# materight/non-rigid-object-tracking

Measured on NVIDIA B200. Metric: PC masker frames/sec at 1080p, higher is better.
Workload: dtype u8/f64

## Files before the change

non-rigid-object-tracking_b200/csrc/pcm_api.cu:

```cuda
#include "../../include/pcm_b200.h"
#include "pcm_kernels.cuh"
#include "pcm_score_variants.h"
#include "pcm_quickshift.cuh"
#include "pcm_forest_fit.cuh"
#include "pcm_prior.cuh"
#include "pcm_slic.cuh"
#include "pcm_host.h"

#include <cudaTypedefs.h>
#include <cub/device/device_radix_sort.cuh>
#include <cub/device/device_scan.cuh>

#include <algorithm>
#include <atomic>
#include <cmath>
#include <cstdarg>
#include <cstddef>
#include <cstdio>
#include <cstring>
#include <cstdlib>
#include <string>
#include <utility>
#include <vector>

// ... 383 lines not shown
    g.PS = (g.RS * (MAX_TILE_H + 2 * n) + 127) / 128 * 128;
    return g;
}

static int int_threshold(double thr) {
    auto le = [&](int v) { return (double)(float)((double)v / 255.0) <= thr; };
    if (!(thr >= -1.0)) return le(-1) ? -1 : -2;
    int t = thr >= 1.5 ? 255 : (int)floor(thr * 255.0);
    t = std::min(std::max(t, -2), 255);
    while (t < 255 && le(t + 1)) ++t;
    while (t >= -1 && !le(t)) --t;
    return t;
}

struct EncTree {
    std::vector<NodeT> nodes;
    std::vector<double> values;
    int n_leaf = 0;
    int depth = 0;
};

struct Encoder {
    const Geom& g;
    const int32_t* feature;
    const double* threshold;
    const int32_t* left;
    const int32_t* right;
    const double* value1;
    int n;
    std::vector<int> tint;
    EncTree out;
    std::string err;

    int skip(int i) const {
        while (left[i] != -1 && tint[i] < -1) i = right[i];
        return i;
    }
    bool run() {
        tint.assign(n, 0);
        for (int i = 0; i < n; ++i) {
            if (left[i] == -1) continue;
            if (left[i] < 0 || left[i] >= n || right[i] < 0 || right[i] >= n) { err = "child index out of range"; return false; }
            if (feature[i] < 0 || feature[i] >= g.F) { err = "feature index out of range"; return false; }
            tint[i] = int_threshold(threshold[i]);
        }
        struct Item { int node, entry, depth; };
        std::vector<Item> queue;
        queue.push_back({skip(0), 0, 0});
        out.nodes.assign(1, make_node(0, 0, 0));
        out.values.assign(1, 0.0);
        const int vplane = 3 * g.n_spaces;
        size_t visited = 0;
        for (size_t qi = 0; qi < queue.size(); ++qi) {
            const Item it = queue[qi];
            if (++visited > (size_t)n + 1) { err = "tree is not a tree"; return false; }
            const int i = it.node;
            if (left[i] == -1) {
                out.nodes[it.entry] = make_node(0u, LEAF_THR, (unsigned)it.entry);
                out.values[it.entry] = value1[i];
                out.n_leaf++;
                out.depth = std::max(out.depth, it.depth);
                continue;
            }
            const int f = feature[i];
            const int q = f / (3 * g.K), rem = f % (3 * g.K), k = rem / 3, ch = rem % 3;
            int dr, dc;
            star_tap(k, dr, dc);
            int plane = 3 * q + ch;
            int thr = tint[i];
            if (thr == -1) { plane = vplane; thr = 0; }
            const unsigned off = (unsigned)(plane * g.PS + (dr + g.n) * g.RS + (dc + g.HX));
            if (off >= (1u << 16)) { err = "tap offset overflow"; return false; }
            const int child = (int)out.nodes.size();
            out.nodes.resize(child + 2, make_node(0, 0, 0));
            out.values.resize(child + 2, 0.0);
            out.nodes[it.entry] = make_node(off, (unsigned)thr, (unsigned)child);
            queue.push_back({skip(left[i]), child, it.depth + 1});
            queue.push_back({skip(right[i]), child + 1, it.depth + 1});
        }
        return true;
    }
};

constexpr int N_SCORE_VARIANTS = 3 * N_SCORE_VARIANTS_PER_PPT;
static const ScoreVariant& score_variant(int i) {
    const ScoreVariant* t = i < N_SCORE_VARIANTS_PER_PPT ? score_variants_ppt6()
                          : i < 2 * N_SCORE_VARIANTS_PER_PPT ? score_variants_ppt7() : score_variants_ppt8();
    return t[i % N_SCORE_VARIANTS_PER_PPT];
}
static const ScoreVariant& pick_score_variant(bool smem, int depth, int ppt) {
    int dyn = -1;
    for (int i = 0; i < N_SCORE_VARIANTS; ++i) {
        const ScoreVariant& v = score_variant(i);
        if (v.smem != smem || v.ppt != ppt) continue;
        if (v.depth == depth) return v;
        if (v.depth == 0) dyn = i;
    }
    return score_variant(dyn);
}

typedef void (*ResidualFn)(const int16_t*, long long, int, int, const double*, const double*, double*);
namespace { extern const ResidualFn pca_residual_kernels[PCM_MAX_PCA_COMPONENTS]; }

struct DeviceShared {
    std::mutex m;
    bool ready = false;
    int sm_count = 0, max_smem_optin = 0;
    PFN_cuTensorMapEncodeTiled_v12000 encode_tiled = nullptr;
    ColorTables h_tables;
    ColorTables* d_tables = nullptr;
};
static DeviceShared& device_shared(int device) {
    static DeviceShared table[64];
    return table[device & 63];
}

extern "C" int pcm_abi_version(void) { return PCM_ABI_VERSION; }
extern "C" const char* pcm_last_error(void) { return g_last_error.c_str(); }

extern "C" int pcm_create(int device, pcm_handle** out) {
    if (!out) return fail(PCM_E_INVALID, "pcm_create: out is NULL");
    *out = nullptr;
    int count = 0;
    cudaError_t e = cudaGetDeviceCount(&count);
    if (e != cudaSuccess || count == 0)
        return fail(PCM_E_CUDA, "pcm_create: no CUDA device (%s); this library has no CPU path",
                    e == cudaSuccess ? "device count 0" : cudaGetErrorString(e));
    if (device < 0 || device >= count) return fail(PCM_E_INVALID, "pcm_create: device %d out of range [0,%d)", device, count);
    CUDA_TRY(cudaSetDevice(device));
    DeviceShared& ds = device_shared(device);
    {
        std::lock_guard<std::mutex> lk(ds.m);
        if (!ds.ready) {
            CUDA_TRY(cudaDeviceGetAttribute(&ds.sm_count, cudaDevAttrMultiProcessorCount, device));
            CUDA_TRY(cudaDeviceGetAttribute(&ds.max_smem_optin, cudaDevAttrMaxSharedMemoryPerBlockOptin, device));
            void* fn = nullptr;
            cudaDriverEntryPointQueryResult qres;
            CUDA_TRY(cudaGetDriverEntryPointByVersion("cuTensorMapEncodeTiled", &fn, 12000, cudaEnableDefault, &qres));
            if (qres != cudaDriverEntryPointSuccess || !fn)
                return fail(PCM_E_CUDA, "pcm_create: driver does not provide cuTensorMapEncodeTiled");
            ds.encode_tiled = reinterpret_cast<PFN_cuTensorMapEncodeTiled_v12000>(fn);
            build_tables(ds.h_tables);
            CUDA_TRY(cudaMalloc(&ds.d_tables, sizeof(ColorTables)));
            CUDA_TRY(cudaMemcpy(ds.d_tables, &ds.h_tables, sizeof(ColorTables), cudaMemcpyHostToDevice));
            for (int i = 0; i < N_SCORE_VARIANTS; ++i)
                CUDA_TRY(cudaFuncSetAttribute(score_variant(i).fn, cudaFuncAttributeMaxDynamicSharedMemorySize, ds.max_smem_optin));
            CUDA_TRY(cudaFuncSetAttribute(qs_density_kernel<false>, cudaFuncAttributeMaxDynamicSharedMemorySize, ds.max_smem_optin));
            CUDA_TRY(cudaFuncSetAttribute(qs_density_kernel<true>, cudaFuncAttributeMaxDynamicSharedMemorySize, ds.max_smem_optin));
            CUDA_TRY(cudaFuncSetAttribute(qs_parent_kernel, cudaFuncAttributeMaxDynamicSharedMemorySize, ds.max_smem_optin));
            CUDA_TRY(cudaFuncSetAttribute(novelty_kernel, cudaFuncAttributeMaxDynamicSharedMemorySize, ds.max_smem_optin));
            for (ResidualFn fn : pca_residual_kernels)
                CUDA_TRY(cudaFuncSetAttribute(fn, cudaFuncAttributeMaxDynamicSharedMemorySize, ds.max_smem_optin));
            ds.ready = true;
        }
    }
    pcm_handle* h = new pcm_handle();
    h->device = device;
    h->sm_count = ds.sm_count;
    h->max_smem_optin = ds.max_smem_optin;
    h->encode_tiled = ds.encode_tiled;
    h->d_tables = ds.d_tables;
    h->h_tables = ds.h_tables;
    CUDA_TRY(cudaStreamCreateWithFlags(&h->own_stream, cudaStreamNonBlocking));
    h->stream = h->own_stream;
    CUDA_TRY(h->err_buf.reserve(sizeof(int)));
    h->d_err = h->err_buf.as<int>();
    CUDA_TRY(cudaMemsetAsync(h->d_err, 0, sizeof(int), h->stream));
    *out = h;
    return PCM_OK;
}

namespace {
const ResidualFn pca_residual_kernels[PCM_MAX_PCA_COMPONENTS] = {
    pca_residual_kernel<1>, pca_residual_kernel<2>, pca_residual_kernel<3>, pca_residual_kernel<4>,
    pca_residual_kernel<5>, pca_residual_kernel<6>, pca_residual_kernel<7>, pca_residual_kernel<8>};
}

// ... 1767 lines not shown
```

non-rigid-object-tracking_b200/csrc/pcm_score.cuh:

```cuda
#pragma once
#include "pcm_device.cuh"
#include <cuda.h>

namespace pcm {

typedef uint2 NodeT;
__host__ __device__ inline NodeT make_node(unsigned tap, unsigned thr, unsigned left) { return make_uint2((tap << 16) | thr, left); }
__host__ __device__ inline unsigned node_tap(const NodeT& n) { return n.x >> 16; }
__host__ __device__ inline unsigned node_thr(const NodeT& n) { return n.x & 0xffffu; }
__host__ __device__ inline unsigned node_left(const NodeT& n) { return n.y; }
__host__ __device__ inline void node_set_left(NodeT& n, unsigned v) { n.y = v; }
constexpr unsigned LEAF_THR = 0xffffu;
constexpr unsigned NODE_BYTES = sizeof(NodeT);

struct DevForest {
    const NodeT* nodes;
    const double* leaves;
    const int4* trees;
    int n_trees, n_nodes, n_leaves;
};

constexpr int MAX_TOP_TREES = 48;
struct TopNodes {
    NodeT n[MAX_TOP_TREES][3];
// ... 117 lines not shown
                    convert((w3[(3 * j) / 4] >> (8 * ((3 * j) % 4))) & 0xff, (w3[(3 * j + 1) / 4] >> (8 * ((3 * j + 1) % 4))) & 0xff,
                            (w3[(3 * j + 2) / 4] >> (8 * ((3 * j + 2) % 4))) & 0xff, j, out);
                    valid |= 1u << (8 * j);
                }
            }
        }
        uint8_t* dst = a.planes + (long long)r * a.pitch + c0;
#pragma unroll
        for (int p = 0; p < NOUT; ++p)
            if (p < nch) *reinterpret_cast<uint32_t*>(dst + p * a.plane_stride) = out[p];
        *reinterpret_cast<uint32_t*>(dst + nch * a.plane_stride) = valid;
        w3[0] = nx[0]; w3[1] = nx[1]; w3[2] = nx[2];
        r = rn; g = gn;
        rn += dr; gn += dg;
        if (gn >= groups_per_row) { gn -= groups_per_row; ++rn; }
    }
    if (a.early) grid_dependency_wait();
}


__device__ __forceinline__ uint32_t smem_u32(const void* p) { return (uint32_t)__cvta_generic_to_shared(p); }

__device__ __forceinline__ void mbar_init(uint32_t bar, uint32_t count) {
    asm volatile("mbarrier.init.shared::cta.b64 [%0], %1;" ::"r"(bar), "r"(count) : "memory");
}
__device__ __forceinline__ void mbar_expect_tx(uint32_t bar, uint32_t bytes) {
    asm volatile("mbarrier.arrive.expect_tx.shared::cta.b64 _, [%0], %1;" ::"r"(bar), "r"(bytes) : "memory");
}
__device__ __forceinline__ void mbar_wait(uint32_t bar, uint32_t parity) {
    uint32_t done;
    do {
        asm volatile(
            "{\n\t.reg .pred p;\n\t"
            "mbarrier.try_wait.parity.shared::cta.b64 p, [%1], %2;\n\t"
            "selp.u32 %0, 1, 0, p;\n\t}"
            : "=r"(done) : "r"(bar), "r"(parity) : "memory");
    } while (!done);
}
__device__ __forceinline__ void tma_load_3d(uint32_t dst, const void* tmap, int x, int y, int z, uint32_t bar) {
    asm volatile(
        "cp.async.bulk.tensor.3d.shared::cluster.global.mbarrier::complete_tx::bytes [%0], [%1, {%2, %3, %4}], [%5];"
        ::"r"(dst), "l"(tmap), "r"(x), "r"(y), "r"(z), "r"(bar) : "memory");
}
__device__ __forceinline__ uint2 lds_v2(uint32_t a) {
    uint2 v;
    asm volatile("ld.shared.v2.u32 {%0, %1}, [%2];" : "=r"(v.x), "=r"(v.y) : "r"(a));
    return v;
}
__device__ __forceinline__ NodeT lds_node(uint32_t a) { return lds_v2(a); }
__device__ __forceinline__ uint32_t lds_u16(uint32_t a) {
    uint32_t v;
    asm volatile("ld.shared.u16 %0, [%1];" : "=r"(v) : "r"(a));
    return v;
}
__device__ __forceinline__ uint32_t lds_u8(uint32_t a) {
    uint32_t v;
    asm volatile("ld.shared.u8 %0, [%1];" : "=r"(v) : "r"(a));
    return v;
}
__device__ __forceinline__ double lds_f64(uint32_t a) {
    double v;
    asm volatile("ld.shared.f64 %0, [%1];" : "=d"(v) : "r"(a));
    return v;
}

struct SegAcc {
    const int32_t* labels;
    int n_labels;
    double thr;
    double* sum;
    double* asum;
    int* area;
    int* rmin;
    int* rmax;
    int* cmin;
    int* cmax;
    int* err;
};

__device__ __forceinline__ double contribution(double p1, double sa, double thr) {
    return __dsub_rn(p1, __dsub_rn(fmax(sa, thr), thr));
}

__device__ __forceinline__ void segment_flush(const SegAcc& s, int lab, double sm, double as, int cnt, int r0, int r1, int col) {
    const int lane = threadIdx.x & 31;
    unsigned todo = __ballot_sync(0xffffffffu, lab >= 0);
    while (todo) {
        const int leader = __ffs(todo) - 1;
        const int L = __shfl_sync(0xffffffffu, lab, leader);
        const bool mine = (lab == L);
        const unsigned members = __ballot_sync(0xffffffffu, mine);
        double x = mine ? sm : 0.0, y = mine ? as : 0.0;
#pragma unroll
        for (int o = 16; o > 0; o >>= 1) {
            x += __shfl_xor_sync(0xffffffffu, x, o);
            y += __shfl_xor_sync(0xffffffffu, y, o);
        }
        const int n = __reduce_add_sync(0xffffffffu, mine ? cnt : 0);
        const int lo = __reduce_min_sync(0xffffffffu, mine ? r0 : 0x7fffffff);
        const int hi = __reduce_max_sync(0xffffffffu, mine ? r1 : -1);
        const int cl = __reduce_min_sync(0xffffffffu, mine ? col : 0x7fffffff);
        const int ch = __reduce_max_sync(0xffffffffu, mine ? col : -1);
        if (lane == leader) {
            atomicAdd(s.sum + L, x);
            atomicAdd(s.asum + L, y);
            atomicAdd(s.area + L, n);
            atomicMin(s.rmin + L, lo);
            atomicMax(s.rmax + L, hi);
            atomicMin(s.cmin + L, cl);
            atomicMax(s.cmax + L, ch);
        }
        todo &= ~members;
    }
}

struct ScoreArgs {
    int cw, ch;
    int tiles_x, tiles_y;
    int tile_y0;
    Geom g;
    unsigned* tile_counter;
    DevForest f0, f1;
    TopNodes top0, top1;
    int depth;
    int blend;
    double w0, w1;
    int novelty;
    DevPCA pca0, pca1;
    double* p1_out;
    double* sa_out;
    SegAcc seg;
    const double* nov_in;
};

__device__ __forceinline__ bool goes_right(uint32_t v, uint32_t x) { return v > (x & 0xffffu); }

__device__ __forceinline__ uint32_t step_child(uint32_t left, uint32_t v, uint32_t x) {
    asm("{\n\t.reg .pred p;\n\t.reg .b32 t;\n\tand.b32 t, %2, 0xffff;\n\tsetp.gt.u32 p, %1, t;\n\t@p add.u32 %0, %0, 8;\n\t}"
        : "+r"(left) : "r"(v), "r"(x));
    return left;
}

template <bool SM, int DEPTH, int PIX_PER_THREAD>
__device__ __forceinline__ void traverse_forest(const uint32_t nodes_s, const uint32_t leaves_s,
                                                const uint8_t* __restrict__ nodes_g,
                                                const uint8_t* __restrict__ leaves_g,
                                                const int4* __restrict__ trees, const int n_trees, const int depth,
                                                const TopNodes& top,
                                                const uint32_t (&pix)[PIX_PER_THREAD],
                                                double (&acc)[PIX_PER_THREAD]) {
    const uint32_t base = SM ? nodes_s : 0u;
    const uint32_t vdelta = leaves_s - nodes_s;

    auto descend = [&](uint32_t (&ref)[PIX_PER_THREAD], const int levels) {
        auto level = [&]() {
            NodeT nd[PIX_PER_THREAD];
            uint32_t v[PIX_PER_THREAD];
#pragma unroll
            for (int g = 0; g < PIX_PER_THREAD; ++g)
                nd[g] = SM ? lds_node(ref[g]) : __ldg(reinterpret_cast<const NodeT*>(nodes_g + ref[g]));
#pragma unroll
            for (int g = 0; g < PIX_PER_THREAD; ++g) v[g] = lds_u8(pix[g] + node_tap(nd[g]));
#pragma unroll
            for (int g = 0; g < PIX_PER_THREAD; ++g) ref[g] = step_child(node_left(nd[g]), v[g], nd[g].x);
        };
        if (DEPTH > 0) {
#pragma unroll
            for (int l = 0; l < levels; ++l) level();
        } else {
#pragma unroll 1
            for (int l = 0; l < levels; ++l) level();
        }
#pragma unroll
        for (int g = 0; g < PIX_PER_THREAD; ++g) {
            const double leaf = SM ? lds_f64(ref[g] + vdelta)
                                   : __ldg(reinterpret_cast<const double*>(leaves_g + ref[g]));
            acc[g] = __dadd_rn(acc[g], leaf);
        }
    };

    const int n_top = n_trees < MAX_TOP_TREES ? n_trees : MAX_TOP_TREES;
    const int rest = DEPTH > 0 ? (DEPTH > 2 ? DEPTH - 2 : 0) : (depth > 2 ? depth - 2 : 0);
#pragma unroll 1
    for (int t = 0; t < n_top; ++t) {
        const NodeT e0 = top.n[t][0], eL = top.n[t][1], eR = top.n[t][2];
        uint32_t ref[PIX_PER_THREAD], v[PIX_PER_THREAD], x1[PIX_PER_THREAD];
#pragma unroll
        for (int g = 0; g < PIX_PER_THREAD; ++g) v[g] = lds_u8(pix[g] + node_tap(e0));
#pragma unroll
        for (int g = 0; g < PIX_PER_THREAD; ++g) {
            const bool right = goes_right(v[g], e0.x);
            x1[g] = right ? eR.x : eL.x;
            ref[g] = (right ? node_left(eR) : node_left(eL)) + base;
        }
#pragma unroll
        for (int g = 0; g < PIX_PER_THREAD; ++g) v[g] = lds_u8(pix[g] + (x1[g] >> 16));
#pragma unroll
        for (int g = 0; g < PIX_PER_THREAD; ++g) ref[g] = step_child(ref[g], v[g], x1[g]);
        descend(ref, DEPTH > 0 ? (DEPTH > 2 ? DEPTH - 2 : 0) : rest);
    }
#pragma unroll 1
    for (int t = n_top; t < n_trees; ++t) {
        uint32_t ref[PIX_PER_THREAD];
#pragma unroll
        for (int g = 0; g < PIX_PER_THREAD; ++g) ref[g] = (uint32_t)trees[t].x + base;
        descend(ref, DEPTH > 0 ? DEPTH : depth);
    }
}

template <int NCH, int PIX_PER_THREAD>
__device__ __forceinline__ void novelty_error(const double* __restrict__ comp, const double* __restrict__ comp255,
                                              const double* __restrict__ mean, const uint32_t* __restrict__ noff,
                                              const double mdc, const int* __restrict__ sp, const Geom& g, const bool interior,
                                              const uint32_t (&pix)[PIX_PER_THREAD], double (&err)[PIX_PER_THREAD]) {
    const int vplane = NCH * g.PS;
    double t[PIX_PER_THREAD];
#pragma unroll
    for (int i = 0; i < PIX_PER_THREAD; ++i) t[i] = 0.0;
#pragma unroll 1
    for (int pass = 0; pass < 2; ++pass) {
#pragma unroll 1
        for (int k = 0; k < g.K; ++k) {
            unsigned ok = (1u << PIX_PER_THREAD) - 1u;
            if (!interior) {
                const int so = sp[k];
                ok = 0;
#pragma unroll
                for (int i = 0; i < PIX_PER_THREAD; ++i) ok |= (unsigned)(lds_u8(pix[i] + vplane + so) != 0) << i;
            }
#pragma unroll
            for (int p = 0; p < NCH; ++p) {
                const int it = k * NCH + p;
                const uint32_t off = noff[it];
                if (pass == 0) {
                    const double c255 = comp255[it];
#pragma unroll
                    for (int i = 0; i < PIX_PER_THREAD; ++i) {
                        const double v = ((ok >> i) & 1u) ? u8_to_double(lds_u8(pix[i] + off)) : -1.0;
                        t[i] = fma(v, c255, t[i]);
                    }
                } else {
                    const double c = comp[it], mu = mean[it];
#pragma unroll
                    for (int i = 0; i < PIX_PER_THREAD; ++i) {
                        const double v = ((ok >> i) & 1u) ? u8_to_double(lds_u8(pix[i] + off)) : -1.0;
                        err[i] += fabs(fma(v, 1.0 / 255.0, -fma(t[i], c, mu)));
                    }
                }
            }
        }
        if (pass == 0) {
#pragma unroll
            for (int i = 0; i < PIX_PER_THREAD; ++i) t[i] -= mdc;
        }
    }
}

__device__ __forceinline__ double blend2(double a, double b, double w0, double w1) {
    return __ddiv_rn(__dadd_rn(__dmul_rn(a, w0), __dmul_rn(b, w1)), __dadd_rn(w0, w1));
}

#ifndef PCM_U8_TILE_BUFS
#define PCM_U8_TILE_BUFS 2
#endif
constexpr int N_TILE_BUF = PCM_U8_TILE_BUFS;

struct ScoreSmem {
    uint32_t tiles, bars, sched, sp, f0_nodes, f0_leaves, f0_trees, f1_nodes, f1_leaves, f1_trees, pca0, pca1, nov_off, total;
};

__host__ __device__ inline uint32_t align_up(uint32_t v, uint32_t a) { return (v + a - 1) / a * a; }

__host__ __device__ inline ScoreSmem score_smem_layout(const Geom& g, const DevForest& f0, const DevForest& f1,
                                                       bool blend, bool novelty, bool forest_smem) {
    ScoreSmem s;
    uint32_t o = 0;
    const int nbuf = N_TILE_BUF;
    s.tiles = o;  o = align_up(o + nbuf * align_up(g.n_planes * g.PS, 128), 128);
    s.bars = o;   o += 8 * nbuf;
    s.sched = o;  o = align_up(o + 4 * nbuf, 16);
    s.sp = o;     o = align_up(o + 4 * g.K, 16);
    s.f0_nodes = s.f0_leaves = s.f1_nodes = s.f1_leaves = 0;
    s.f0_trees = o;  o = align_up(o + 16 * f0.n_trees, 16);
    s.f1_trees = o;
    if (blend) o = align_up(o + 16 * f1.n_trees, 16);
    if (forest_smem) {
        s.f0_nodes = o;  o = align_up(o + NODE_BYTES * f0.n_nodes, 16);
        s.f0_leaves = o; o = align_up(o + 8 * f0.n_nodes, 16);
        if (blend) {
            s.f1_nodes = o;  o = align_up(o + NODE_BYTES * f1.n_nodes, 16);
            s.f1_leaves = o; o = align_up(o + 8 * f1.n_nodes, 16);
        }
    }
    s.pca0 = s.pca1 = s.nov_off = 0;
    if (novelty) {
        s.pca0 = o; o = align_up(o + 24 * g.F, 16);
        if (blend) { s.pca1 = o; o = align_up(o + 24 * g.F, 16); }
        s.nov_off = o; o = align_up(o + 4 * g.F, 16);
    }
    s.total = o;
    return s;
}

template <typename T>
__device__ __forceinline__ void copy_to_smem(T* dst, const T* __restrict__ src, int n) {
    for (int i = threadIdx.x; i < n; i += NTHREADS) dst[i] = src[i];
}

__device__ __forceinline__ void stage_nodes(uint8_t* dst, const NodeT* __restrict__ src, int n) {
    const uint32_t base = smem_u32(dst);
    for (int i = threadIdx.x; i < n; i += NTHREADS) {
        NodeT nd = src[i];
        node_set_left(nd, node_left(nd) + base);
        reinterpret_cast<NodeT*>(dst)[i] = nd;
    }
}

template <bool FOREST_SMEM, int DEPTH, int PIX_PER_THREAD>
__global__ void __launch_bounds__(NTHREADS, PCM_MIN_CTAS) score_kernel(const __grid_constant__ CUtensorMap tmap, const ScoreArgs a) {
    extern __shared__ __align__(128) uint8_t smem[];
    const Geom& g = a.g;
    const ScoreSmem L = score_smem_layout(g, a.f0, a.f1, a.blend != 0, a.novelty != 0 && !a.nov_in, FOREST_SMEM);
    constexpr int TILE_H = ROW_GROUPS * PIX_PER_THREAD;
    const int PH = TILE_H + 2 * g.n;
    const uint32_t tile_bytes = align_up(g.n_planes * g.PS, 128);
    const uint32_t tiles_s = smem_u32(smem + L.tiles);
    const uint32_t bars_s = smem_u32(smem + L.bars);
    volatile int* sched = reinterpret_cast<volatile int*>(smem + L.sched);
    int* sp = reinterpret_cast<int*>(smem + L.sp);
    const int tid = threadIdx.x, lane = tid & 31, warp = tid >> 5;
    const int n_tiles = a.tiles_x * a.tiles_y;
    const uint32_t box_bytes = (uint32_t)(g.n_planes * g.RS * PH);

    auto issue = [&](int buf) {
        const int t = (int)atomicAdd(a.tile_counter, 1u);
        sched[buf] = t;
        if (t < n_tiles) {
            const uint32_t bar = bars_s + 8 * buf;
            mbar_expect_tx(bar, box_bytes);
            const int x = (t % a.tiles_x) * TILE_W - g.HX, y = (a.tile_y0 + t / a.tiles_x) * TILE_H - g.n;
            for (int pl = 0; pl < g.n_planes; ++pl)
                tma_load_3d(tiles_s + buf * tile_bytes + pl * g.PS, &tmap, x, y, pl, bar);
        }
    };

    for (int k = tid; k < g.K; k += NTHREADS) {
        int dr, dc;
        star_tap(k, dr, dc);
        sp[k] = (dr + g.n) * g.RS + (dc + g.HX);
    }
    copy_to_smem(reinterpret_cast<int4*>(smem + L.f0_trees), a.f0.trees, a.f0.n_trees);
    if (a.blend) copy_to_smem(reinterpret_cast<int4*>(smem + L.f1_trees), a.f1.trees, a.f1.n_trees);
    const int4* f0t = reinterpret_cast<const int4*>(smem + L.f0_trees);
    const int4* f1t = reinterpret_cast<const int4*>(smem + L.f1_trees);
    if (FOREST_SMEM) {
        stage_nodes(smem + L.f0_nodes, a.f0.nodes, a.f0.n_nodes);
        copy_to_smem(reinterpret_cast<double*>(smem + L.f0_leaves), a.f0.leaves, a.f0.n_nodes);
        if (a.blend) {
            stage_nodes(smem + L.f1_nodes, a.f1.nodes, a.f1.n_nodes);
            copy_to_smem(reinterpret_cast<double*>(smem + L.f1_leaves), a.f1.leaves, a.f1.n_nodes);
        }
    }
    const double *p0c = nullptr, *p0c255 = nullptr, *p0m = nullptr, *p1c = nullptr, *p1c255 = nullptr, *p1m = nullptr;
    const uint32_t* noff = reinterpret_cast<const uint32_t*>(smem + L.nov_off);
    if (a.novelty && !a.nov_in) {
        const int nch = 3 * g.n_spaces;
        double* d0 = reinterpret_cast<double*>(smem + L.pca0);
        double* d1 = reinterpret_cast<double*>(smem + L.pca1);
        uint32_t* no = reinterpret_cast<uint32_t*>(smem + L.nov_off);
        for (int it = tid; it < g.F; it += NTHREADS) {
            const int k = it / nch, p = it - k * nch;
            const int f = (p / 3) * 3 * g.K + 3 * k + (p % 3);
            int dr, dc;
            star_tap(k, dr, dc);
            no[it] = (uint32_t)(p * g.PS + (dr + g.n) * g.RS + (dc + g.HX));
            d0[it] = a.pca0.comp[f]; d0[g.F + it] = a.pca0.comp255[f]; d0[2 * g.F + it] = a.pca0.mean[f];
            if (a.blend) { d1[it] = a.pca1.comp[f]; d1[g.F + it] = a.pca1.comp255[f]; d1[2 * g.F + it] = a.pca1.mean[f]; }
        }
        p0c = d0; p0c255 = d0 + g.F; p0m = d0 + 2 * g.F;
        p1c = d1; p1c255 = d1 + g.F; p1m = d1 + 2 * g.F;
    }
    grid_dependency_wait();
    grid_launch_dependents();
    if (tid == 0) {
        for (int b = 0; b < N_TILE_BUF; ++b) mbar_init(bars_s + 8 * b, 1);
        asm volatile("fence.mbarrier_init.release.cluster;" ::: "memory");
        asm volatile("fence.proxy.async.shared::cta;" ::: "memory");
        if (N_TILE_BUF > 1) issue(0);
    }

    __syncthreads();

    const uint32_t f0n_s = smem_u32(smem + L.f0_nodes), f0l_s = smem_u32(smem + L.f0_leaves);
    const uint32_t f1n_s = smem_u32(smem + L.f1_nodes), f1l_s = smem_u32(smem + L.f1_leaves);
    const uint8_t* f0n_g = reinterpret_cast<const uint8_t*>(a.f0.nodes);
    const uint8_t* f0l_g = reinterpret_cast<const uint8_t*>(a.f0.leaves);
    const uint8_t* f1n_g = reinterpret_cast<const uint8_t*>(a.f1.nodes);
    const uint8_t* f1l_g = reinterpret_cast<const uint8_t*>(a.f1.leaves);

    const int col = (warp & 1) * 32 + lane;
    const int row0 = (warp >> 1) * PIX_PER_THREAD;
    uint32_t phase = 0;
    for (int buf = 0;; buf = (N_TILE_BUF > 1) ? (buf ^ 1) : 0) {
        if (N_TILE_BUF == 1) {
            if (tid == 0) issue(0);
            __syncthreads();
        }
        const int tile = sched[buf];
        if (tile >= n_tiles) break;
        if (N_TILE_BUF > 1 && tid == 0) issue(buf ^ 1);
        mbar_wait(bars_s + 8 * buf, (phase >> buf) & 1u);
        phase ^= 1u << buf;

        const int tx0 = (tile % a.tiles_x) * TILE_W, ty0 = (a.tile_y0 + tile / a.tiles_x) * TILE_H;
        const int ox = tx0 + col;
        uint32_t pix[PIX_PER_THREAD];
#pragma unroll
        for (int i = 0; i < PIX_PER_THREAD; ++i) pix[i] = tiles_s + buf * tile_bytes + (row0 + i) * g.RS + col;

        int lab[PIX_PER_THREAD];
#pragma unroll
        for (int i = 0; i < PIX_PER_THREAD; ++i) {
            const int oy = ty0 + row0 + i;
            lab[i] = (ox < a.cw && oy < a.ch) ? __ldg(a.seg.labels + (size_t)oy * a.cw + ox) : -1;
        }

        double p[PIX_PER_THREAD];
#pragma unroll
        for (int i = 0; i < PIX_PER_THREAD; ++i) p[i] = 0.0;
        traverse_forest<FOREST_SMEM, DEPTH, PIX_PER_THREAD>(f0n_s, f0l_s, f0n_g, f0l_g, f0t, a.f0.n_trees, a.depth, a.top0, pix, p);
        const double T0 = (double)a.f0.n_trees;
#pragma unroll
        for (int i = 0; i < PIX_PER_THREAD; ++i) p[i] = __ddiv_rn(p[i], T0);
        if (a.blend) {
            double q[PIX_PER_THREAD];
#pragma unroll
            for (int i = 0; i < PIX_PER_THREAD; ++i) q[i] = 0.0;
            traverse_forest<FOREST_SMEM, DEPTH, PIX_PER_THREAD>(f1n_s, f1l_s, f1n_g, f1l_g, f1t, a.f1.n_trees, a.depth, a.top1, pix, q);
            const double T1 = (double)a.f1.n_trees;
#pragma unroll
            for (int i = 0; i < PIX_PER_THREAD; ++i) p[i] = blend2(p[i], __ddiv_rn(q[i], T1), a.w0, a.w1);
        }
        double e[PIX_PER_THREAD];
#pragma unroll
        for (int i = 0; i < PIX_PER_THREAD; ++i) e[i] = 0.0;
        if (a.novelty && a.nov_in) {
#pragma unroll
            for (int i = 0; i < PIX_PER_THREAD; ++i) {
                const int oy = ty0 + row0 + i;
                if (ox < a.cw && oy < a.ch) e[i] = __ldg(a.nov_in + (size_t)oy * a.cw + ox);
            }
        } else if (a.novelty) {
            const bool interior = ox >= g.n && ox + g.n < a.cw && ty0 + row0 >= g.n && ty0 + row0 + PIX_PER_THREAD - 1 + g.n < a.ch;
            auto run = [&](const double* c, const double* c255, const double* mu, double mdc, double (&out)[PIX_PER_THREAD]) {
                switch (g.n_spaces) {
                    case 1: novelty_error<3, PIX_PER_THREAD>(c, c255, mu, noff, mdc, sp, g, interior, pix, out); break;
                    case 2: novelty_error<6, PIX_PER_THREAD>(c, c255, mu, noff, mdc, sp, g, interior, pix, out); break;
                    default: novelty_error<9, PIX_PER_THREAD>(c, c255, mu, noff, mdc, sp, g, interior, pix, out); break;
                }
            };
            run(p0c, p0c255, p0m, a.pca0.mean_dot_comp, e);
            if (a.blend) {
                double e1[PIX_PER_THREAD];
#pragma unroll
                for (int i = 0; i < PIX_PER_THREAD; ++i) e1[i] = 0.0;
                run(p1c, p1c255, p1m, a.pca1.mean_dot_comp, e1);
#pragma unroll
                for (int i = 0; i < PIX_PER_THREAD; ++i) e[i] = blend2(e[i], e1[i], a.w0, a.w1);
            }
        }
        int run_lab = -1, run_cnt = 0, run_r0 = 0, run_r1 = 0;
        double run_sum = 0.0, run_abs = 0.0;
#pragma unroll
        for (int i = 0; i < PIX_PER_THREAD; ++i) {
            const int oy = ty0 + row0 + i;
            int l = lab[i];
            if (ox < a.cw && oy < a.ch) {
                const size_t o = (size_t)oy * a.cw + ox;
                if (a.p1_out) {
                    a.p1_out[o] = p[i];
                    if (a.novelty && !a.nov_in) a.sa_out[o] = e[i];
                }
                if (l < 0 || l >= a.seg.n_labels) { *a.seg.err = 1; l = -1; }
            }
            const bool change = (l != run_lab) && run_lab >= 0;
            if (__any_sync(0xffffffffu, change)) {
                segment_flush(a.seg, change ? run_lab : -1, run_sum, run_abs, run_cnt, run_r0, run_r1, ox);
                if (change) run_lab = -1;
            }
            if (l >= 0) {
                const double d = contribution(p[i], e[i], a.seg.thr);
                if (run_lab < 0) { run_lab = l; run_cnt = 0; run_sum = 0.0; run_abs = 0.0; run_r0 = oy; }
                run_sum += d; run_abs += fabs(d); run_cnt++; run_r1 = oy;
            }
        }
        segment_flush(a.seg, run_lab, run_sum, run_abs, run_cnt, run_r0, run_r1, ox);
        __syncthreads();
    }
}

}
```

non-rigid-object-tracking_b200/csrc/pcm_score_inst.cu:

```cuda
#include "pcm_score_variants.h"

#ifndef PCM_PPT
#error "compile with -DPCM_PPT=6, 7 or 8"
#endif
#define PCM_STR2(x) #x
#define PCM_STR(x) PCM_STR2(x)
#define PCM_CAT2(a, b) a##b
#define PCM_CAT(a, b) PCM_CAT2(a, b)
#define PCM_SV(S, D) {S, D, PCM_PPT, score_kernel<S, D, PCM_PPT>, "score_kernel<" #S "," #D "," PCM_STR(PCM_PPT) ">"}

namespace pcm {

static_assert(PCM_PPT >= MIN_PPT && PCM_PPT <= MAX_PPT, "tile height outside the range the shared-memory layout is sized for");

const ScoreVariant* PCM_CAT(score_variants_ppt, PCM_PPT)() {
    static const ScoreVariant v[N_SCORE_VARIANTS_PER_PPT] = {
        PCM_SV(true, 5),  PCM_SV(true, 7),  PCM_SV(true, 10),  PCM_SV(true, 0),
        PCM_SV(false, 5), PCM_SV(false, 7), PCM_SV(false, 10), PCM_SV(false, 0),
    };
    return v;
}

}
```

non-rigid-object-tracking_b200/csrc/pcm_score_variants.h:

```cpp
#pragma once
#include "pcm_score.cuh"

namespace pcm {

typedef void (*ScoreFn)(const CUtensorMap, const ScoreArgs);
struct ScoreVariant {
    bool smem;
    int depth;
    int ppt;
    ScoreFn fn;
    const char* name;
};
constexpr int N_SCORE_VARIANTS_PER_PPT = 8;
const ScoreVariant* score_variants_ppt6();
const ScoreVariant* score_variants_ppt7();
const ScoreVariant* score_variants_ppt8();

}
```

non-rigid-object-tracking_b200/pcm/build.py:

```python
import os
import subprocess
import sys

PKG = os.path.dirname(os.path.dirname(os.path.abspath(__file__)))
CSRC = os.path.join(PKG, "csrc")
LIB = os.environ.get("PCM_LIB_PATH") or os.path.join(PKG, "libpcm_b200.so")
UNITS = [("pcm_api.cu", [], "pcm_api.o"),
         ("pcm_score_inst.cu", ["-DPCM_PPT=6"], "pcm_score_ppt6.o"),
         ("pcm_score_inst.cu", ["-DPCM_PPT=7"], "pcm_score_ppt7.o"),
         ("pcm_score_inst.cu", ["-DPCM_PPT=8"], "pcm_score_ppt8.o"),
         ("pcm_host_simd.cpp", [], "pcm_host_simd.o"),
         ("pcm_felzenszwalb.cpp", [], "pcm_felzenszwalb.o"),
         ("pcm_slic.cpp", [], "pcm_slic.o")]
DEPS = ["pcm_api.cu", "pcm_score_inst.cu", "pcm_score_variants.h", "pcm_score.cuh", "pcm_kernels.cuh", "pcm_device.cuh", "pcm_host.h",
        "pcm_host_simd.cpp", "pcm_felzenszwalb.cpp", "pcm_slic.cpp", "pcm_slic.cuh", "pcm_quickshift.cuh", "pcm_forest_fit.cuh", "pcm_prior.cuh",
        os.path.join("..", "..", "include", "pcm_b200.h")]

NVCC_FLAGS = [
    "-gencode", "arch=compute_100a,code=sm_100a",
    "-O3", "-std=c++17", "-lineinfo",
    "-Xcompiler", "-fPIC", "-Xcompiler", "-pthread", "-Xcompiler", "-ffp-contract=off",
    "-Xptxas", "-v",
]


def needs_build():
    if not os.path.isfile(LIB):
        return True
    t = os.path.getmtime(LIB)
    return any(os.path.getmtime(os.path.join(CSRC, d)) > t for d in DEPS)


def build(force=False, verbose=False):
    if not force and not needs_build():
        return LIB
    nvcc = os.environ.get("NVCC", "nvcc")
    extra = os.environ.get("PCM_BUILD_DEFS", "").split()
    objdir = os.path.join(PKG, "build", "obj" if LIB.endswith("libpcm_b200.so") else "obj_" + os.path.basename(LIB))
    os.makedirs(objdir, exist_ok=True)
    procs = []
    for src, defs, obj in UNITS:
        cmd = [nvcc] + NVCC_FLAGS + extra + defs + ["-c", "-o", os.path.join(objdir, obj), os.path.join(CSRC, src)]
        procs.append((cmd, subprocess.Popen(cmd, stdout=subprocess.PIPE, stderr=subprocess.PIPE, text=True)))
    log = []
    for cmd, pr in procs:
        out, err = pr.communicate()
        log.append(out + err)
        if verbose or pr.returncode != 0:
            sys.stderr.write(out + err)
        if pr.returncode != 0:
            for _, other in procs:
                if other.poll() is None:
                    other.kill()
            raise RuntimeError("nvcc failed (%d): %s" % (pr.returncode, " ".join(cmd)))
    link = [nvcc, "-gencode", "arch=compute_100a,code=sm_100a", "-shared", "-Xcompiler", "-pthread", "-o", LIB] + \
           [os.path.join(objdir, obj) for _, _, obj in UNITS]
    res = subprocess.run(link, capture_output=True, text=True)
    if verbose or res.returncode != 0:
        sys.stderr.write(res.stdout + res.stderr)
    if res.returncode != 0:
        raise RuntimeError("link failed (%d): %s" % (res.returncode, " ".join(link)))
    if LIB.endswith("libpcm_b200.so"):
        with open(os.path.join(PKG, "build", "ptxas_info.txt"), "w") as f:
            f.write("".join(l for text in log for l in text.splitlines(True) if "Compile time" not in l))
    return LIB


if __name__ == "__main__":
    print(build(force="--force" in sys.argv, verbose=True))
```

Before: 7064.

## Add row-walk forest traversal sharing tree paths across 8 horizontal pixels

Adds a score-kernel variant for 8 pixels per thread in which each thread owns 8 horizontally adjacent pixels and descends each tree once for the whole group. A packed SIMD byte comparison tests all 8 pixels against a node threshold together and falls back to per-pixel descent only when the group diverges. It is meant to cut redundant node loads and per-pixel traversal work where neighbouring pixels take the same path, and it also vectorises the label loads. The cost is extra test arithmetic, different segment-flush reduction patterns, and divergence where pixels split. It becomes the default for ppt=8, and an environment variable restores the old pixel walk.

```diff
diff --git a/non-rigid-object-tracking_b200/csrc/pcm_api.cu b/non-rigid-object-tracking_b200/csrc/pcm_api.cu
--- a/non-rigid-object-tracking_b200/csrc/pcm_api.cu
+++ b/non-rigid-object-tracking_b200/csrc/pcm_api.cu
@@ -489,17 +489,19 @@
     }
 };
 
-constexpr int N_SCORE_VARIANTS = 3 * N_SCORE_VARIANTS_PER_PPT;
+constexpr int N_SCORE_VARIANTS = 4 * N_SCORE_VARIANTS_PER_PPT;
 static const ScoreVariant& score_variant(int i) {
-    const ScoreVariant* t = i < N_SCORE_VARIANTS_PER_PPT ? score_variants_ppt6()
-                          : i < 2 * N_SCORE_VARIANTS_PER_PPT ? score_variants_ppt7() : score_variants_ppt8();
-    return t[i % N_SCORE_VARIANTS_PER_PPT];
+    static const ScoreVariant* (*const tables[4])() = {score_variants_ppt6, score_variants_ppt7, score_variants_ppt8,
+                                                       score_variants_ppt8_pixel};
+    return tables[i / N_SCORE_VARIANTS_PER_PPT]()[i % N_SCORE_VARIANTS_PER_PPT];
 }
 static const ScoreVariant& pick_score_variant(bool smem, int depth, int ppt) {
+    static const bool pixel_walk = [] { const char* e = getenv("PCM_K1_WALK"); return e && strcmp(e, "pixel") == 0; }();
+    const bool row_walk = ppt == MAX_PPT && !pixel_walk;
     int dyn = -1;
     for (int i = 0; i < N_SCORE_VARIANTS; ++i) {
         const ScoreVariant& v = score_variant(i);
-        if (v.smem != smem || v.ppt != ppt) continue;
+        if (v.smem != smem || v.ppt != ppt || v.row_walk != row_walk) continue;
         if (v.depth == depth) return v;
         if (v.depth == 0) dyn = i;
     }
diff --git a/non-rigid-object-tracking_b200/csrc/pcm_score.cuh b/non-rigid-object-tracking_b200/csrc/pcm_score.cuh
--- a/non-rigid-object-tracking_b200/csrc/pcm_score.cuh
+++ b/non-rigid-object-tracking_b200/csrc/pcm_score.cuh
@@ -223,7 +223,8 @@
     return __dsub_rn(p1, __dsub_rn(fmax(sa, thr), thr));
 }
 
-__device__ __forceinline__ void segment_flush(const SegAcc& s, int lab, double sm, double as, int cnt, int r0, int r1, int col) {
+__device__ __forceinline__ void segment_flush(const SegAcc& s, int lab, double sm, double as, int cnt, int r0, int r1,
+                                              int c0, int c1) {
     const int lane = threadIdx.x & 31;
     unsigned todo = __ballot_sync(0xffffffffu, lab >= 0);
     while (todo) {
@@ -240,8 +241,8 @@
         const int n = __reduce_add_sync(0xffffffffu, mine ? cnt : 0);
         const int lo = __reduce_min_sync(0xffffffffu, mine ? r0 : 0x7fffffff);
         const int hi = __reduce_max_sync(0xffffffffu, mine ? r1 : -1);
-        const int cl = __reduce_min_sync(0xffffffffu, mine ? col : 0x7fffffff);
-        const int ch = __reduce_max_sync(0xffffffffu, mine ? col : -1);
+        const int cl = __reduce_min_sync(0xffffffffu, mine ? c0 : 0x7fffffff);
+        const int ch = __reduce_max_sync(0xffffffffu, mine ? c1 : -1);
         if (lane == leader) {
             atomicAdd(s.sum + L, x);
             atomicAdd(s.asum + L, y);
@@ -346,6 +347,109 @@
 #pragma unroll
         for (int g = 0; g < PIX_PER_THREAD; ++g) ref[g] = (uint32_t)trees[t].x + base;
         descend(ref, DEPTH > 0 ? DEPTH : depth);
+    }
+}
+
+
+__device__ __forceinline__ bool row_test(uint32_t pix0, uint32_t x, bool& right) {
+    static_assert((LEAF_THR & 0xffu) == 0xffu, "the packed test reads a leaf's threshold from its low byte");
+    const uint32_t at = pix0 + (x >> 16), b = at & ~7u;
+    const uint2 lo = lds_v2(b), hi = lds_v2(b + 8);
+    const bool up = (at & 4u) != 0;
+    const uint32_t w0 = up ? lo.y : lo.x, w1 = up ? hi.x : lo.y, w2 = up ? hi.y : hi.x;
+    const uint32_t r0 = __funnelshift_r(w0, w1, at * 8u), r1 = __funnelshift_r(w1, w2, at * 8u);
+    const uint32_t k = (~x & 0xffu) * 0x00010001u, m = 0x00ff00ffu, c = 0x01000100u;
+    const uint32_t s0 = (r0 & m) + k, s1 = __byte_perm(r0, 0u, 0x4341) + k;
+    const uint32_t s2 = (r1 & m) + k, s3 = __byte_perm(r1, 0u, 0x4341) + k;
+    right = (s0 & s1 & s2 & s3 & c) == c;
+    return !right && ((s0 | s1 | s2 | s3) & c) != 0u;
+}
+
+template <bool SM, int DEPTH>
+__device__ __forceinline__ void traverse_forest_row(const uint32_t nodes_s, const uint32_t leaves_s,
+                                                    const uint8_t* __restrict__ nodes_g,
+                                                    const uint8_t* __restrict__ leaves_g,
+                                                    const int4* __restrict__ trees, const int n_trees, const int depth,
+                                                    const TopNodes& top, const uint32_t pix0, double (&acc)[8]) {
+    constexpr int P = 8;
+    const uint32_t base = SM ? nodes_s : 0u;
+    const uint32_t vdelta = leaves_s - nodes_s;
+    auto node = [&](uint32_t r) -> NodeT { return SM ? lds_node(r) : __ldg(reinterpret_cast<const NodeT*>(nodes_g + r)); };
+    auto leaf = [&](uint32_t r) -> double {
+        return SM ? lds_f64(r + vdelta) : __ldg(reinterpret_cast<const double*>(leaves_g + r));
+    };
+    auto level = [&](uint32_t& ref, int& rem, const int left) {
+        const NodeT nd = node(ref);
+        bool right;
+        const bool mixed = row_test(pix0, nd.x, right);
+        const bool walking = rem == 0;
+        ref = (walking && !mixed) ? node_left(nd) + (right ? NODE_BYTES : 0u) : ref;
+        rem = (walking && mixed) ? left : rem;
+    };
+    auto finish = [&](const uint32_t ref, const int rem) {
+        if (rem != 0) {
+            uint32_t r[P];
+#pragma unroll
+            for (int g = 0; g < P; ++g) r[g] = ref;
+#pragma unroll 1
+            for (int l = 0; l < rem; ++l) {
+                NodeT nd[P];
+                uint32_t v[P];
+#pragma unroll
+                for (int g = 0; g < P; ++g) nd[g] = node(r[g]);
+#pragma unroll
+                for (int g = 0; g < P; ++g) v[g] = lds_u8(pix0 + g + node_tap(nd[g]));
+#pragma unroll
+                for (int g = 0; g < P; ++g) r[g] = step_child(node_left(nd[g]), v[g], nd[g].x);
+            }
+#pragma unroll
+            for (int g = 0; g < P; ++g) acc[g] = __dadd_rn(acc[g], leaf(r[g]));
+        } else {
+            const double v = leaf(ref);
+#pragma unroll
+            for (int g = 0; g < P; ++g) acc[g] = __dadd_rn(acc[g], v);
+        }
+    };
+
+    const int D = DEPTH > 0 ? DEPTH : depth;
+    const int n_top = n_trees < MAX_TOP_TREES ? n_trees : MAX_TOP_TREES;
+    const int top_levels = D > 2 ? D : 2;
+#pragma unroll 1
+    for (int t = 0; t < n_top; ++t) {
+        const NodeT e0 = top.n[t][0], eL = top.n[t][1], eR = top.n[t][2];
+        uint32_t ref;
+        int rem = 0;
+        bool r0, r1;
+        if (row_test(pix0, e0.x, r0)) {
+            rem = top_levels;
+            ref = (uint32_t)trees[t].x + base;
+        } else if (row_test(pix0, r0 ? eR.x : eL.x, r1)) {
+            rem = top_levels - 1;
+            ref = node_left(e0) + base + (r0 ? NODE_BYTES : 0u);
+        } else {
+            ref = (r0 ? node_left(eR) : node_left(eL)) + base + (r1 ? NODE_BYTES : 0u);
+        }
+        if (DEPTH > 0) {
+#pragma unroll
+            for (int l = 2; l < DEPTH; ++l) level(ref, rem, DEPTH - l);
+        } else {
+#pragma unroll 1
+            for (int l = 2; l < D && rem == 0; ++l) level(ref, rem, D - l);
+        }
+        finish(ref, rem);
+    }
+#pragma unroll 1
+    for (int t = n_top; t < n_trees; ++t) {
+        uint32_t ref = (uint32_t)trees[t].x + base;
+        int rem = 0;
+        if (DEPTH > 0) {
+#pragma unroll
+            for (int l = 0; l < DEPTH; ++l) level(ref, rem, DEPTH - l);
+        } else {
+#pragma unroll 1
+            for (int l = 0; l < D && rem == 0; ++l) level(ref, rem, D - l);
+        }
+        finish(ref, rem);
     }
 }
 
@@ -457,8 +561,9 @@
     }
 }
 
-template <bool FOREST_SMEM, int DEPTH, int PIX_PER_THREAD>
+template <bool FOREST_SMEM, int DEPTH, int PIX_PER_THREAD, bool ROW_WALK>
 __global__ void __launch_bounds__(NTHREADS, PCM_MIN_CTAS) score_kernel(const __grid_constant__ CUtensorMap tmap, const ScoreArgs a) {
+    static_assert(!ROW_WALK || PIX_PER_THREAD == 8, "the row walk maps 8 rows x 4 lanes of 8 pixels onto a warp");
     extern __shared__ __align__(128) uint8_t smem[];
     const Geom& g = a.g;
     const ScoreSmem L = score_smem_layout(g, a.f0, a.f1, a.blend != 0, a.novelty != 0 && !a.nov_in, FOREST_SMEM);
@@ -539,8 +644,10 @@
     const uint8_t* f1n_g = reinterpret_cast<const uint8_t*>(a.f1.nodes);
     const uint8_t* f1l_g = reinterpret_cast<const uint8_t*>(a.f1.leaves);
 
-    const int col = (warp & 1) * 32 + lane;
-    const int row0 = (warp >> 1) * PIX_PER_THREAD;
+    constexpr int DX = ROW_WALK ? 1 : 0, DY = ROW_WALK ? 0 : 1;
+    const int col = (warp & 1) * 32 + (ROW_WALK ? (lane & 3) * 8 : lane);
+    const int row0 = (warp >> 1) * PIX_PER_THREAD + (ROW_WALK ? lane >> 2 : 0);
+    const uint32_t pstep = ROW_WALK ? 1u : (uint32_t)g.RS;
     uint32_t phase = 0;
     for (int buf = 0;; buf = (N_TILE_BUF > 1) ? (buf ^ 1) : 0) {
         if (N_TILE_BUF == 1) {
@@ -554,22 +661,39 @@
         phase ^= 1u << buf;
 
         const int tx0 = (tile % a.tiles_x) * TILE_W, ty0 = (a.tile_y0 + tile / a.tiles_x) * TILE_H;
-        const int ox = tx0 + col;
+        const int ox = tx0 + col, oy = ty0 + row0;
+        const uint32_t pix0 = tiles_s + buf * tile_bytes + row0 * g.RS + col;
         uint32_t pix[PIX_PER_THREAD];
 #pragma unroll
-        for (int i = 0; i < PIX_PER_THREAD; ++i) pix[i] = tiles_s + buf * tile_bytes + (row0 + i) * g.RS + col;
+        for (int i = 0; i < PIX_PER_THREAD; ++i) pix[i] = pix0 + i * pstep;
+        auto inside = [&](int i) { return ox + DX * i < a.cw && oy + DY * i < a.ch; };
+        auto at = [&](int i) { return (size_t)(oy + DY * i) * a.cw + (ox + DX * i); };
 
         int lab[PIX_PER_THREAD];
-#pragma unroll
-        for (int i = 0; i < PIX_PER_THREAD; ++i) {
-            const int oy = ty0 + row0 + i;
-            lab[i] = (ox < a.cw && oy < a.ch) ? __ldg(a.seg.labels + (size_t)oy * a.cw + ox) : -1;
+        bool lab_vec = false;
+        if constexpr (ROW_WALK) {
+            const int4* l4 = reinterpret_cast<const int4*>(a.seg.labels + at(0));
+            lab_vec = inside(7) && (reinterpret_cast<uintptr_t>(l4) & 15) == 0;
+            if (lab_vec) {
+                const int4 l0 = __ldg(l4), l1 = __ldg(l4 + 1);
+                lab[0] = l0.x; lab[1] = l0.y; lab[2] = l0.z; lab[3] = l0.w;
+                lab[4] = l1.x; lab[5] = l1.y; lab[6] = l1.z; lab[7] = l1.w;
+            }
+        }
+        if (!lab_vec) {
+#pragma unroll
+            for (int i = 0; i < PIX_PER_THREAD; ++i) lab[i] = inside(i) ? __ldg(a.seg.labels + at(i)) : -1;
         }
 
         double p[PIX_PER_THREAD];
 #pragma unroll
         for (int i = 0; i < PIX_PER_THREAD; ++i) p[i] = 0.0;
-        traverse_forest<FOREST_SMEM, DEPTH, PIX_PER_THREAD>(f0n_s, f0l_s, f0n_g, f0l_g, f0t, a.f0.n_trees, a.depth, a.top0, pix, p);
+        auto forest = [&](uint32_t ns, uint32_t ls, const uint8_t* ng, const uint8_t* lg, const int4* tr, int nt,
+                          const TopNodes& top, double (&acc)[PIX_PER_THREAD]) {
+            if constexpr (ROW_WALK) traverse_forest_row<FOREST_SMEM, DEPTH>(ns, ls, ng, lg, tr, nt, a.depth, top, pix0, acc);
+            else traverse_forest<FOREST_SMEM, DEPTH, PIX_PER_THREAD>(ns, ls, ng, lg, tr, nt, a.depth, top, pix, acc);
+        };
+        forest(f0n_s, f0l_s, f0n_g, f0l_g, f0t, a.f0.n_trees, a.top0, p);
         const double T0 = (double)a.f0.n_trees;
 #pragma unroll
         for (int i = 0; i < PIX_PER_THREAD; ++i) p[i] = __ddiv_rn(p[i], T0);
@@ -577,7 +701,7 @@
             double q[PIX_PER_THREAD];
 #pragma unroll
             for (int i = 0; i < PIX_PER_THREAD; ++i) q[i] = 0.0;
-            traverse_forest<FOREST_SMEM, DEPTH, PIX_PER_THREAD>(f1n_s, f1l_s, f1n_g, f1l_g, f1t, a.f1.n_trees, a.depth, a.top1, pix, q);
+            forest(f1n_s, f1l_s, f1n_g, f1l_g, f1t, a.f1.n_trees, a.top1, q);
             const double T1 = (double)a.f1.n_trees;
 #pragma unroll
             for (int i = 0; i < PIX_PER_THREAD; ++i) p[i] = blend2(p[i], __ddiv_rn(q[i], T1), a.w0, a.w1);
@@ -587,12 +711,11 @@
         for (int i = 0; i < PIX_PER_THREAD; ++i) e[i] = 0.0;
         if (a.novelty && a.nov_in) {
 #pragma unroll
-            for (int i = 0; i < PIX_PER_THREAD; ++i) {
-                const int oy = ty0 + row0 + i;
-                if (ox < a.cw && oy < a.ch) e[i] = __ldg(a.nov_in + (size_t)oy * a.cw + ox);
-            }
+            for (int i = 0; i < PIX_PER_THREAD; ++i)
+                if (inside(i)) e[i] = __ldg(a.nov_in + at(i));
         } else if (a.novelty) {
-            const bool interior = ox >= g.n && ox + g.n < a.cw && ty0 + row0 >= g.n && ty0 + row0 + PIX_PER_THREAD - 1 + g.n < a.ch;
+            constexpr int LAST = PIX_PER_THREAD - 1;
+            const bool interior = ox >= g.n && ox + DX * LAST + g.n < a.cw && oy >= g.n && oy + DY * LAST + g.n < a.ch;
             auto run = [&](const double* c, const double* c255, const double* mu, double mdc, double (&out)[PIX_PER_THREAD]) {
                 switch (g.n_spaces) {
                     case 1: novelty_error<3, PIX_PER_THREAD>(c, c255, mu, noff, mdc, sp, g, interior, pix, out); break;
@@ -610,14 +733,16 @@
                 for (int i = 0; i < PIX_PER_THREAD; ++i) e[i] = blend2(e[i], e1[i], a.w0, a.w1);
             }
         }
-        int run_lab = -1, run_cnt = 0, run_r0 = 0, run_r1 = 0;
+        int run_lab = -1, run_cnt = 0, run_i0 = 0, run_i1 = 0;
         double run_sum = 0.0, run_abs = 0.0;
+        auto flush = [&](int l) {
+            segment_flush(a.seg, l, run_sum, run_abs, run_cnt, oy + DY * run_i0, oy + DY * run_i1, ox + DX * run_i0, ox + DX * run_i1);
+        };
 #pragma unroll
         for (int i = 0; i < PIX_PER_THREAD; ++i) {
-            const int oy = ty0 + row0 + i;
             int l = lab[i];
-            if (ox < a.cw && oy < a.ch) {
-                const size_t o = (size_t)oy * a.cw + ox;
+            if (inside(i)) {
+                const size_t o = at(i);
                 if (a.p1_out) {
                     a.p1_out[o] = p[i];
                     if (a.novelty && !a.nov_in) a.sa_out[o] = e[i];
@@ -626,16 +751,16 @@
             }
             const bool change = (l != run_lab) && run_lab >= 0;
             if (__any_sync(0xffffffffu, change)) {
-                segment_flush(a.seg, change ? run_lab : -1, run_sum, run_abs, run_cnt, run_r0, run_r1, ox);
+                flush(change ? run_lab : -1);
                 if (change) run_lab = -1;
             }
             if (l >= 0) {
                 const double d = contribution(p[i], e[i], a.seg.thr);
-                if (run_lab < 0) { run_lab = l; run_cnt = 0; run_sum = 0.0; run_abs = 0.0; run_r0 = oy; }
-                run_sum += d; run_abs += fabs(d); run_cnt++; run_r1 = oy;
-            }
-        }
-        segment_flush(a.seg, run_lab, run_sum, run_abs, run_cnt, run_r0, run_r1, ox);
+                if (run_lab < 0) { run_lab = l; run_cnt = 0; run_sum = 0.0; run_abs = 0.0; run_i0 = i; }
+                run_sum += d; run_abs += fabs(d); run_cnt++; run_i1 = i;
+            }
+        }
+        flush(run_lab);
         __syncthreads();
     }
 }
diff --git a/non-rigid-object-tracking_b200/csrc/pcm_score_inst.cu b/non-rigid-object-tracking_b200/csrc/pcm_score_inst.cu
--- a/non-rigid-object-tracking_b200/csrc/pcm_score_inst.cu
+++ b/non-rigid-object-tracking_b200/csrc/pcm_score_inst.cu
@@ -3,17 +3,33 @@
 #ifndef PCM_PPT
 #error "compile with -DPCM_PPT=6, 7 or 8"
 #endif
+#ifndef PCM_PIXEL_WALK
+#define PCM_PIXEL_WALK 0
+#endif
+#if PCM_PPT == 8 && !PCM_PIXEL_WALK
+#define PCM_ROW_WALK true
+#define PCM_WALK_NAME "row"
+#else
+#define PCM_ROW_WALK false
+#define PCM_WALK_NAME "pixel"
+#endif
 #define PCM_STR2(x) #x
 #define PCM_STR(x) PCM_STR2(x)
 #define PCM_CAT2(a, b) a##b
 #define PCM_CAT(a, b) PCM_CAT2(a, b)
-#define PCM_SV(S, D) {S, D, PCM_PPT, score_kernel<S, D, PCM_PPT>, "score_kernel<" #S "," #D "," PCM_STR(PCM_PPT) ">"}
+#define PCM_SV(S, D) {S, D, PCM_PPT, PCM_ROW_WALK, score_kernel<S, D, PCM_PPT, PCM_ROW_WALK>, \
+                      "score_kernel<" #S "," #D "," PCM_STR(PCM_PPT) "," PCM_WALK_NAME ">"}
 
 namespace pcm {
 
 static_assert(PCM_PPT >= MIN_PPT && PCM_PPT <= MAX_PPT, "tile height outside the range the shared-memory layout is sized for");
 
+#if PCM_PIXEL_WALK
+static_assert(PCM_PPT == 8, "only the 32-row tile has a second walk");
+const ScoreVariant* score_variants_ppt8_pixel() {
+#else
 const ScoreVariant* PCM_CAT(score_variants_ppt, PCM_PPT)() {
+#endif
     static const ScoreVariant v[N_SCORE_VARIANTS_PER_PPT] = {
         PCM_SV(true, 5),  PCM_SV(true, 7),  PCM_SV(true, 10),  PCM_SV(true, 0),
         PCM_SV(false, 5), PCM_SV(false, 7), PCM_SV(false, 10), PCM_SV(false, 0),
diff --git a/non-rigid-object-tracking_b200/csrc/pcm_score_variants.h b/non-rigid-object-tracking_b200/csrc/pcm_score_variants.h
--- a/non-rigid-object-tracking_b200/csrc/pcm_score_variants.h
+++ b/non-rigid-object-tracking_b200/csrc/pcm_score_variants.h
@@ -8,6 +8,7 @@
     bool smem;
     int depth;
     int ppt;
+    bool row_walk;
     ScoreFn fn;
     const char* name;
 };
@@ -15,5 +16,6 @@
 const ScoreVariant* score_variants_ppt6();
 const ScoreVariant* score_variants_ppt7();
 const ScoreVariant* score_variants_ppt8();
+const ScoreVariant* score_variants_ppt8_pixel();
 
 }
diff --git a/non-rigid-object-tracking_b200/pcm/build.py b/non-rigid-object-tracking_b200/pcm/build.py
--- a/non-rigid-object-tracking_b200/pcm/build.py
+++ b/non-rigid-object-tracking_b200/pcm/build.py
@@ -9,6 +9,7 @@
          ("pcm_score_inst.cu", ["-DPCM_PPT=6"], "pcm_score_ppt6.o"),
          ("pcm_score_inst.cu", ["-DPCM_PPT=7"], "pcm_score_ppt7.o"),
          ("pcm_score_inst.cu", ["-DPCM_PPT=8"], "pcm_score_ppt8.o"),
+         ("pcm_score_inst.cu", ["-DPCM_PPT=8", "-DPCM_PIXEL_WALK=1"], "pcm_score_ppt8_pixel.o"),
          ("pcm_host_simd.cpp", [], "pcm_host_simd.o"),
          ("pcm_felzenszwalb.cpp", [], "pcm_felzenszwalb.o"),
          ("pcm_slic.cpp", [], "pcm_slic.o")]
```

New measurement: 5069 (median of 6 runs). 28.2% lower.
